# HydraRadio/hydra-pspec

Measured on NVIDIA B200. Metric: baseline-Gibbs-iterations/sec at Nfreq=384, Ntimes=1024, Nfg=32 on 1/8 B200, higher is better.
Workload: dtype f64 (complex128)

## Files before the change

### hydra_pspec_b200/_lib.py

```python
import ctypes as C
import os
from pathlib import Path

import numpy as np

_HERE = Path(__file__).resolve().parent
LIB_PATH = Path(os.environ.get("HP_LIB_PATH", _HERE / "csrc" / "libhydra_pspec_b200.so"))

HP_RNG_INJECTED, HP_RNG_PHILOX = 0, 1
HP_KEEP_CR, HP_KEEP_FG, HP_KEEP_CHISQ = 1, 2, 4
(HP_BUF_PS, HP_BUF_LNPOST, HP_BUF_CR, HP_BUF_FG, HP_BUF_CHISQ, HP_BUF_LAST_CR, HP_BUF_LAST_FG,
 HP_BUF_PS_CUR) = range(8)
HP_NUM_KERNEL_CLASSES = 6
HP_SUMMARY_CR, HP_SUMMARY_FG = 1, 2


class HPConfig(C.Structure):
    _fields_ = [
        ("device", C.c_int), ("nchains", C.c_int), ("ntimes", C.c_int), ("nfreqs", C.c_int),
        ("nmodes", C.c_int), ("rng_mode", C.c_int), ("cg_compat", C.c_int), ("refresh_omega", C.c_int),
        ("keep", C.c_int), ("max_iters", C.c_int), ("general_basis0", C.c_int), ("profile", C.c_int), ("substreams", C.c_int), ("dense_noise", C.c_int),
        ("force_dense_transforms", C.c_int), ("force_dense_solve", C.c_int), ("time_flags", C.c_int),
        ("ring_iters", C.c_int), ("seed", C.c_uint64), ("stream", C.c_void_p),
    ]
# ... 31 lines not shown
    "hp_engine_kernel_ms": (C.c_int, [C.c_void_p, C.c_void_p, C.c_void_p, C.c_int]),
    "hp_engine_set_substreams": (C.c_int, [C.c_void_p, C.c_int]),
    "hp_engine_set_chain_ids": (C.c_int, [C.c_void_p, C.c_void_p]),
    "hp_engine_set_profile": (C.c_int, [C.c_void_p, C.c_int]),
    "hp_engine_launch_count": (C.c_longlong, [C.c_void_p]),
    "hp_engine_set_summary": (C.c_int, [C.c_void_p, C.c_int, C.c_int, C.c_int]),
    "hp_engine_read_summary": (C.c_int, [C.c_void_p, C.c_int, C.c_int, C.c_void_p, C.c_void_p, C.c_size_t,
                                         C.POINTER(C.c_int)]),
    "hp_engine_set_summary_batched": (C.c_int, [C.c_void_p, C.c_int, C.c_int, C.c_int, C.c_int]),
    "hp_engine_read_summary_mcse": (C.c_int, [C.c_void_p, C.c_int, C.c_int, C.c_void_p, C.c_void_p, C.c_size_t,
                                              C.POINTER(C.c_int)]),
    "hp_engine_pt_form": (C.c_int, [C.c_void_p, C.POINTER(C.c_int), C.POINTER(C.c_int)]),
    "hp_kernel_class_name": (C.c_char_p, [C.c_int]),
    "hp_sample_S": (C.c_int, [C.c_int, C.c_int, C.c_int, C.c_void_p, C.c_void_p, C.c_void_p, C.c_void_p]),
    "hp_fourier_operator": (C.c_int, [C.c_int, C.c_int, C.c_void_p]),
    "hp_eigh_batch": (C.c_int, [C.c_int, C.c_int, C.c_int, C.c_void_p, C.c_void_p, C.c_void_p, C.c_void_p]),
    "hp_test_zgemm": (C.c_int, [C.c_int, C.c_int, C.c_int, C.c_void_p, C.c_int, C.c_int, C.c_void_p, C.c_int,
                                C.c_int, C.c_void_p, C.c_void_p]),
    "hp_test_chol_solve": (C.c_int, [C.c_int, C.c_int, C.c_int, C.c_void_p, C.c_void_p, C.c_void_p, C.c_void_p,
                                     C.c_int, C.c_void_p, C.c_void_p, C.c_void_p]),
    "hp_test_solve3": (C.c_int, [C.c_int, C.c_int, C.c_int, C.c_int, C.c_void_p, C.c_void_p, C.c_void_p, C.c_void_p,
                                 C.c_int, C.c_int, C.c_void_p, C.c_void_p]),
    "hp_test_solve3_schedule": (C.c_int, [C.c_int, C.c_void_p, C.c_void_p, C.POINTER(C.c_int), C.POINTER(C.c_int)]),
    "hp_fp64_peak_tflops": (C.c_double, [C.c_int, C.c_double]),
    "hp_release_cached_memory": (None, []),
    "hp_pinned_alloc": (C.c_void_p, [C.c_size_t]),
    "hp_pinned_free": (None, [C.c_void_p]),
    "hp_last_error": (C.c_char_p, []),
    "hp_version": (C.c_char_p, []),
}
EXPORTED_SYMBOLS = tuple(_SIGNATURES)


def lib():
    global _lib
    if _lib is None:
        if not LIB_PATH.exists():
            raise HydraLibError(
                f"{LIB_PATH} not found: build it with hydra_pspec_b200/csrc/build.sh "
                "(hydra_pspec_b200 has no CPU fallback)")
        L = C.CDLL(os.fspath(LIB_PATH))
        for name, (res, args) in _SIGNATURES.items():
            fn = getattr(L, name)
            fn.restype = res
            fn.argtypes = args
        _lib = L
# ... 66 lines not shown
```

### hydra_pspec_b200/csrc/hp_engine.cu

```cuda
#include "../../include/hydra_pspec_b200.h"
#include "hp_kernels.cuh"
#include "hp_math.h"

#include <cmath>
#include <cstdio>
#include <cstdlib>
#include <cstring>
#include <mutex>
#include <string>
#include <vector>

namespace {

thread_local std::string g_err;

int fail(int code, const std::string& msg) {
    g_err = msg;
    return code;
}

#define CU_TRY(expr)                                                                              \
    do {                                                                                          \
        cudaError_t _e = (expr);                                                                  \
        if (_e != cudaSuccess)                                                                    \
// ... 1040 lines not shown
        t.B = OFFS(b.Bmat, 2 * n * Np); t.sBk = 1; t.sBj = e->Np; t.bsB = (long long)e->n * e->Np;
        t.C = sf; t.sCi = e->n; t.sCj = 1; t.bsC = o.sf_bs;
        t.M = e->T; t.N = e->n; t.K = e->n; t.accumulate = 0; t.alpha = 1.0; t.batch = sb.nc;
        hp::launch_zgemm(t, sb.st);
        e->prof_end(CLS_TRANSFORM, 1, sb.st);
    }
    e->last_sf = o.sf;
    e->last_sf_bs = o.sf_bs;
    double* fg = o.fg ? o.fg + (size_t)sb.c0 * (size_t)o.fg_bs : nullptr;
    double* chisq = o.chisq ? o.chisq + (size_t)sb.c0 * (size_t)o.chisq_bs : nullptr;

    if (e->fft_ok) {
        e->prof_begin(CLS_POST, sb.st);
        hp::PostFftArgs pa{};
        pa.plan = e->plan; pa.tw = e->tw; pa.tw2 = e->tw2; pa.X = OFFS(e->X, 2 * Tp * Np); pa.lam = OFFS(e->lam, Np); pa.Sf = sf; pa.sf_bs = o.sf_bs;
        pa.Ft = OFFS(e->Ft, 2 * (m ? m : 1) * n); pa.wd = OFFS(e->wd, 2 * Tp * n); pa.w = OFFS(e->w, n); pa.ninvd = OFFS(e->ninvd, n);
        pa.w_bs = e->n; pa.w_ts = 0;
        if (pt) { pa.w = OFFS(e->wT, Tp * n); pa.w_bs = (long long)e->Tp * e->n; pa.w_ts = e->n; }
        pa.fg_out = fg; pa.fg_bs = o.fg_bs; pa.chisq_out = chisq; pa.chisq_bs = o.chisq_bs;
        pa.lnp1 = OFFS(e->lnp1, Tp); pa.Rm = e->cfg.dense_noise ? OFFS(e->Rm, 2 * Tp * n) : nullptr;
        pa.Empart = e->any_flagged ? OFFS(e->Empart, (size_t)e->ntilesE * n) : nullptr;
        pa.Eupart = general ? OFFS(e->Eupart, (size_t)e->ntilesE * n) : nullptr;
        pa.m = e->m; pa.Np = e->Np; pa.T = e->T; pa.Tp = e->Tp; pa.nsys = sb.nc; pa.do_inverse = fused_inverse ? 1 : 0; pa.ktp = e->ktp;
        if (!(e->fft2_ok && pa.do_inverse && !pa.Eupart && hp::launch_post_fft2(pa, e->plan2f, e->plan2r, sb.st)))
            hp::launch_post_fft(pa, sb.st);
        e->prof_end(CLS_POST, 1, sb.st);
        if (e->cfg.dense_noise) enqueue_dense_lnp1(e, sb);
        return;
    }
    e->prof_begin(CLS_POST, sb.st);
    hp::PostArgs pa{};
    pa.Sf = sf; pa.sf_bs = o.sf_bs; pa.X = OFFS(e->X, 2 * Tp * Np); pa.Ft = OFFS(e->Ft, 2 * (m ? m : 1) * n);
    pa.wd = OFFS(e->wd, 2 * Tp * n); pa.w = OFFS(e->w, n); pa.ninvd = OFFS(e->ninvd, n);
    pa.fg_out = fg; pa.fg_bs = o.fg_bs; pa.chisq_out = chisq; pa.chisq_bs = o.chisq_bs;
    pa.Wm = e->any_flagged ? OFFS(e->Wm, 2 * Tp * n) : nullptr; pa.Rm = e->cfg.dense_noise ? OFFS(e->Rm, 2 * Tp * n) : nullptr;
    pa.lnp1 = OFFS(e->lnp1, Tp);
    pa.n = e->n; pa.m = e->m; pa.Np = e->Np; pa.T = e->T; pa.Tp = e->Tp; pa.nsys = sb.nc;
    hp::launch_post(pa, sb.st);
    e->prof_end(CLS_POST, 1, sb.st);
    if (e->cfg.dense_noise) enqueue_dense_lnp1(e, sb);
    if (e->any_flagged || general) {
        e->prof_begin(CLS_TRANSFORM, sb.st);
        int nl2 = 0;
        hp::ZgemmArgs t{};
        t.sAi = e->n; t.sAk = 1; t.bsA = (long long)e->Tp * e->n;
        t.B = e->U; t.sBk = 1; t.sBj = e->n; t.bsB = 0;
// ... 575 lines not shown
```

### hydra_pspec_b200/csrc/hp_fft2.cu

```cuda
#include "hp_kernels.cuh"
#include "hp_math.h"
#include "hp_mma.cuh"
#include <cstdlib>

namespace hp {

namespace {

constexpr int kTP2 = 8;
#ifndef HP_FFT2_CTAS
#define HP_FFT2_CTAS 2
#endif

__device__ __forceinline__ double2 cmul(double2 a, double2 b) { return make_double2(a.x * b.x - a.y * b.y, a.x * b.y + a.y * b.x); }
__device__ __forceinline__ double2 cadd(double2 a, double2 b) { return make_double2(a.x + b.x, a.y + b.y); }
__device__ __forceinline__ double2 csub(double2 a, double2 b) { return make_double2(a.x - b.x, a.y - b.y); }
__device__ __forceinline__ double2 mul_mi(double2 a) { return make_double2(a.y, -a.x); }

template <int R>
__device__ __forceinline__ void butterfly(double2* a);
template <>
__device__ __forceinline__ void butterfly<2>(double2* a) {
    const double2 t = a[1];
    a[1] = csub(a[0], t);
    a[0] = cadd(a[0], t);
}
template <>
__device__ __forceinline__ void butterfly<3>(double2* a) {
    const double S3 = 0.86602540378443864676;
    const double2 t1 = cadd(a[1], a[2]);
    const double2 t2 = make_double2(a[0].x - 0.5 * t1.x, a[0].y - 0.5 * t1.y);
    const double2 t3 = make_double2(S3 * (a[1].y - a[2].y), -S3 * (a[1].x - a[2].x));
// ... 9 lines not shown
template <>
__device__ __forceinline__ void butterfly<6>(double2* a) {
    double2 e[3] = {a[0], a[2], a[4]}, o[3] = {a[3], a[5], a[1]};
    butterfly<3>(e);
    butterfly<3>(o);
    a[0] = cadd(e[0], o[0]); a[3] = csub(e[0], o[0]);
    a[4] = cadd(e[1], o[1]); a[1] = csub(e[1], o[1]);
    a[2] = cadd(e[2], o[2]); a[5] = csub(e[2], o[2]);
}
template <>
__device__ __forceinline__ void butterfly<8>(double2* a) {
    const double H = 0.70710678118654752440;
    double2 e[4] = {a[0], a[2], a[4], a[6]}, o[4] = {a[1], a[3], a[5], a[7]};
    butterfly<4>(e);
    butterfly<4>(o);
    const double2 o1 = make_double2(H * (o[1].x + o[1].y), H * (o[1].y - o[1].x));
    const double2 o2 = mul_mi(o[2]);
    const double2 o3 = make_double2(H * (o[3].y - o[3].x), -H * (o[3].x + o[3].y));
    a[0] = cadd(e[0], o[0]); a[4] = csub(e[0], o[0]);
    a[1] = cadd(e[1], o1);   a[5] = csub(e[1], o1);
    a[2] = cadd(e[2], o2);   a[6] = csub(e[2], o2);
    a[3] = cadd(e[3], o3);   a[7] = csub(e[3], o3);
}

__device__ __forceinline__ int phys(int i) { return i + (i >> 3); }

template <int E, int R, int NS, bool kLoad, bool kStore>
__device__ __forceinline__ void fft_pass(double2 (&v)[E], double2* row, const double2* __restrict__ twt, int lane) {
    constexpr int n = 32 * E, NB = E / R, nb = n / R;
    static_assert(E % R == 0 && nb % 8 == 0, "a lane owns whole butterflies; rows of a butterfly are 8-aligned");
    if (kLoad) {
        const double2* src = row + phys(lane);
#pragma unroll
        for (int u = 0; u < NB; ++u)
#pragma unroll
            for (int r = 0; r < R; ++r) v[u * R + r] = src[36 * u + r * (nb / 8 * 9)];
    }
#pragma unroll
    for (int u = 0; u < NB; ++u) {
        if (NS > 1) {
            const int k = (lane + 32 * u) % NS;
#pragma unroll
            for (int r = 1; r < R; ++r) v[u * R + r] = cmul(v[u * R + r], twt[k * (R - 1) + r - 1]);
        }
        butterfly<R>(&v[u * R]);
    }
// ... 50 lines not shown
    else if (n == 512) { rad[0] = 8; rad[1] = 8; rad[2] = 4; rad[3] = 2; nf = 4; }
    else if (n == 256) { rad[0] = 8; rad[1] = 8; rad[2] = 4; rad[3] = 1; nf = 3; }
    else if (n == 128) { rad[0] = 4; rad[1] = 4; rad[2] = 4; rad[3] = 2; nf = 4; }
    else return false;
    for (int dir = 0; dir < 2; ++dir) {
        FftPlan* p = dir ? rev : fwd;
        p->n = n; p->nf = nf;
        int Ns = 1;
        for (int i = 0; i < nf; ++i) {
            p->radix[i] = dir ? rad[nf - 1 - i] : rad[i];
            p->magic[i] = Ns > 1 ? (uint32_t)((0x100000000ull + (uint64_t)Ns - 1) / (uint64_t)Ns) : 0u;
            Ns *= p->radix[i];
        }
    }
    return true;
}

size_t postfft2_smem_bytes(int n, int m) {
    const int mk = ((m + 3) / 4) * 4;
    const int ld = n + n / 8 + 1;
    return sizeof(double2) * ((size_t)kTP2 * ld + 2 * (size_t)n + (size_t)kTP2 * (((mk + 7) / 8) * 8 + 4)) + 80 * sizeof(double);
}

template <int E, int P0, int P1, int P2, int P3>
__global__ void __launch_bounds__(32 * kTP2, (E >= 16 ? 1 : HP_FFT2_CTAS)) k_post_fft2(PostFftArgs a) {
    constexpr int kThreads = 32 * kTP2;
    constexpr int n = 32 * E, ld = n + n / 8 + 1;
    constexpr int RL = P3 > 1 ? P3 : P2;
    extern __shared__ __align__(16) unsigned char smem_raw[];
    const int m = a.m, mk = ((m + 3) / 4) * 4, ldf = ((mk + 7) / 8) * 8 + 4;
    double2* A = reinterpret_cast<double2*>(smem_raw);
    double2* tw = A + (size_t)kTP2 * ld;
    double2* fs = tw + 2 * (size_t)n;
    double* red = reinterpret_cast<double*>(fs + (size_t)kTP2 * ldf);
    const int sys = blockIdx.y, tile = blockIdx.x, t0 = tile * kTP2;
    const int tid = threadIdx.x, warp = tid >> 5, lane = tid & 31;
    const double* X = a.X + 2 * ((size_t)sys * a.Tp + t0) * a.Np;
    const double* lam = a.lam + (size_t)sys * a.Np;
    const double* w = a.w + (size_t)sys * a.w_bs + (size_t)t0 * a.w_ts;
    const double* nd = a.ninvd + (size_t)sys * n;
    const double* wd = a.wd + 2 * ((size_t)sys * a.Tp + t0) * n;
    double* Sf = a.Sf + 2 * ((size_t)sys * a.sf_bs + (size_t)t0 * n);
    const double2* twg = reinterpret_cast<const double2*>(a.tw);
    const double rsn = rsqrt((double)n);

    {
        const char* wdp = reinterpret_cast<const char*>(wd);
        const size_t bytes = (size_t)min(kTP2, a.T - t0) * n * 16;
        for (size_t off = (size_t)tid * 128; off < bytes; off += kThreads * 128) asm volatile("prefetch.global.L2 [%0];" ::"l"(wdp + off));
    }
    const int t = warp;
    const bool live = t0 + t < a.T;
    double2 v[E];
    {
        constexpr int nb0 = n / P0;
        const double* xr = X + 2 * (size_t)t * a.Np;
#pragma unroll
        for (int e = 0; e < E; ++e) {
            const int u = e / P0, r = e - u * P0;
            const int k = lane + 32 * u + r * nb0;
            double2 y = make_double2(0.0, 0.0);
            double l = 0.0;
            if (live) { y = *reinterpret_cast<const double2*>(xr + 2 * k); l = lam[k]; }
            const double sg = (k & 1) ? -l : l;
            v[e] = make_double2(sg * y.x, -sg * y.y);
        }
    }
    if (a.tw2) {
        const double2* t2 = reinterpret_cast<const double2*>(a.tw2);
        const int cnt = a.Empart ? 2 * n : n;
        for (int e = tid; e < cnt; e += kThreads) tw[e] = t2[e];
    } else {
        build_twiddle_tables<E, P0, P1, P2, P3>(tw, twg, tid, kThreads);
        if (a.Empart) {
            if constexpr (P3 > 1) build_twiddle_tables<E, P3, P2, P1, P0>(tw + n, twg, tid, kThreads);
            else build_twiddle_tables<E, P2, P1, P0, 1>(tw + n, twg, tid, kThreads);
        }
    }
    for (int e = tid; e < kTP2 * ldf; e += kThreads) {
        const int tt = e / ldf, j = e - tt * ldf;
        double2 f = make_double2(0.0, 0.0);
        if (j < m && t0 + tt < a.T) f = *reinterpret_cast<const double2*>(X + 2 * ((size_t)tt * a.Np + n + j));
        fs[e] = f;
        if (j < m && t0 + tt < a.T && a.fg_out)
            *reinterpret_cast<double2*>(a.fg_out + (size_t)sys * a.fg_bs + 2 * ((size_t)(t0 + tt) * m + j)) = f;
    }
    __syncthreads();
    double2* row = A + (size_t)t * ld;
    {
        fft_run<E, P0, P1, P2, P3, true>(v, row, tw, lane);
        constexpr int R = RL, Ns = n / RL;
        const double2 c0 = twg[(int)(((long long)(n / 2) * (n / 2)) % n)];
        __syncwarp();
#pragma unroll
        for (int e = 0; e < E; ++e) {
            const int u = e / R, r = e - u * R;
            const int x = lane + 32 * u + r * Ns;
            double2 o = cmul(v[e], c0);
            const double sg = (x & 1) ? -rsn : rsn;
            o = make_double2(sg * o.x, -sg * o.y);
            row[phys(x)] = o;
            if (live) *reinterpret_cast<double2*>(Sf + 2 * ((size_t)t * n + x)) = o;
        }
    }
    __syncthreads();
    {
        const double* Ft = a.Ft + 2 * (size_t)sys * m * n;
        const int nct = n / 8;
        const int g = lane >> 2, q = lane & 3;
        const bool tlive = t0 + g < a.T;
        const double* wrow = w + (size_t)g * a.w_ts;
        double lnp = 0.0;
        constexpr int kBF = 8;
        double2 bnx[kBF], dnx[2];
        auto load_tile = [&](int ct, double2 (&b)[kBF], double2 (&d)[2]) {
            const int x = 8 * ct + g;
#pragma unroll
            for (int s8 = 0; s8 < kBF; ++s8) {
                const int k = 4 * s8 + q;
                b[s8] = (k < m && ct < nct) ? *reinterpret_cast<const double2*>(Ft + 2 * ((size_t)k * n + x)) : make_double2(0.0, 0.0);
            }
            d[0] = d[1] = make_double2(0.0, 0.0);
            if (tlive && ct < nct) {
                d[0] = *reinterpret_cast<const double2*>(wd + 2 * ((size_t)g * n + 8 * ct + 2 * q));
                d[1] = *reinterpret_cast<const double2*>(wd + 2 * ((size_t)g * n + 8 * ct + 2 * q + 1));
            }
        };
        load_tile(warp, bnx, dnx);
        for (int ct = warp; ct < nct; ct += kTP2) {
            double p1[2] = {0.0, 0.0}, p2[2] = {0.0, 0.0}, p3[2] = {0.0, 0.0};
            const int x0 = 8 * ct + 2 * q;
            double2 bc[kBF];
#pragma unroll
            for (int s8 = 0; s8 < kBF; ++s8) bc[s8] = bnx[s8];
            const double2 d0 = dnx[0], d1 = dnx[1];
            load_tile(ct + kTP2, bnx, dnx);
#pragma unroll
            for (int s8 = 0; s8 < kBF; ++s8) {
                const int k = 4 * s8 + q;
                if (4 * s8 < mk) {
                    const double2 af = fs[(size_t)g * ldf + k];
                    dmma884(p1[0], p1[1], af.x, bc[s8].x);
                    dmma884(p2[0], p2[1], af.y, bc[s8].y);
                    dmma884(p3[0], p3[1], af.x + af.y, bc[s8].x + bc[s8].y);
                }
            }
            for (int kc = 4 * kBF; kc < mk; kc += 4) {
                const int k = kc + q;
                const double2 af = fs[(size_t)g * ldf + k];
                const double2 b = k < m ? *reinterpret_cast<const double2*>(Ft + 2 * ((size_t)k * n + 8 * ct + g)) : make_double2(0.0, 0.0);
                dmma884(p1[0], p1[1], af.x, b.x);
                dmma884(p2[0], p2[1], af.y, b.y);
                dmma884(p3[0], p3[1], af.x + af.y, b.x + b.y);
            }
            const double2 s0 = A[(size_t)g * ld + phys(x0)], s1 = A[(size_t)g * ld + phys(x0 + 1)];
            const double wx0 = (a.w_ts == 0 || tlive) ? wrow[x0] : 0.0, wx1 = (a.w_ts == 0 || tlive) ? wrow[x0 + 1] : 0.0;
            const double n0 = nd[x0], n1 = nd[x0 + 1];
            const double rr0 = d0.x - s0.x - (p1[0] - p2[0]), ri0 = d0.y - s0.y - (p3[0] - p1[0] - p2[0]);
            const double rr1 = d1.x - s1.x - (p1[1] - p2[1]), ri1 = d1.y - s1.y - (p3[1] - p1[1] - p2[1]);
            const double q0 = rr0 * rr0 + ri0 * ri0, q1 = rr1 * rr1 + ri1 * ri1;
            if (tlive) {
                if (a.chisq_out)
                    *reinterpret_cast<double2*>(a.chisq_out + (size_t)sys * a.chisq_bs + (size_t)(t0 + g) * n + x0) = make_double2(q0 * n0, q1 * n1);
                lnp += wx0 * n0 * q0 + wx1 * n1 * q1;
                if (a.Rm) {
                    double* rm = a.Rm + 2 * (((size_t)sys * a.Tp + t0 + g) * n + x0);
                    *reinterpret_cast<double2*>(rm) = make_double2(wx0 * rr0, wx0 * ri0);
                    *reinterpret_cast<double2*>(rm + 2) = make_double2(wx1 * rr1, wx1 * ri1);
                }
            }
            if (a.Empart) {
                A[(size_t)g * ld + phys(x0)] = make_double2(wx0 * s0.x, wx0 * s0.y);
                A[(size_t)g * ld + phys(x0 + 1)] = make_double2(-wx1 * s1.x, -wx1 * s1.y);
            }
        }
        lnp += __shfl_xor_sync(0xffffffffu, lnp, 1);
        lnp += __shfl_xor_sync(0xffffffffu, lnp, 2);
        if (q == 0) red[warp * kTP2 + g] = lnp;
    }
    __syncthreads();
    if (tid < kTP2) {
        double s = 0.0;
        for (int wv = 0; wv < kTP2; ++wv) s += red[wv * kTP2 + tid];
        if (t0 + tid < a.Tp) a.lnp1[(size_t)sys * a.Tp + t0 + tid] = t0 + tid < a.T ? s : 0.0;
    }
    if (a.Empart) {
        if constexpr (P3 > 1) fft_run<E, P3, P2, P1, P0, false>(v, row, tw + n, lane);
        else fft_run<E, P2, P1, P0, 1, false>(v, row, tw + n, lane);
        constexpr int R = P0, Ns = n / P0;
        __syncwarp();
        double* erow = reinterpret_cast<double*>(row);
#pragma unroll
        for (int e = 0; e < E; ++e) {
            const int u = e / R, r = e - u * R;
            erow[lane + 32 * u + r * Ns] = live ? v[e].x * v[e].x + v[e].y * v[e].y : 0.0;
        }
        __syncthreads();
        double* Ep = a.Empart + ((size_t)sys * gridDim.x + tile) * n;
        for (int k = tid; k < n; k += kThreads) {
            double acc = 0.0;
#pragma unroll
            for (int tt = 0; tt < kTP2; ++tt) acc += reinterpret_cast<const double*>(A + (size_t)tt * ld)[k];
            Ep[k] = acc / (double)n;
        }
    }
}

namespace {
template <int E, int P0, int P1, int P2, int P3>
__global__ void __launch_bounds__(256) k_fft2_tables(double2* tw2, const double2* twg) {
    constexpr int n = 32 * E;
    for (int e = threadIdx.x; e < 2 * n; e += 256) tw2[e] = make_double2(0.0, 0.0);
    __syncthreads();
    build_twiddle_tables<E, P0, P1, P2, P3>(tw2, twg, threadIdx.x, 256);
    if constexpr (P3 > 1) build_twiddle_tables<E, P3, P2, P1, P0>(tw2 + n, twg, threadIdx.x, 256);
    else build_twiddle_tables<E, P2, P1, P0, 1>(tw2 + n, twg, threadIdx.x, 256);
}
}

bool launch_fft2_tables(double* tw2, const double* tw, int n, cudaStream_t st) {
    double2* o = reinterpret_cast<double2*>(tw2);
    const double2* t = reinterpret_cast<const double2*>(tw);
    if (n == 128) k_fft2_tables<4, 4, 4, 4, 2><<<1, 256, 0, st>>>(o, t);
    else if (n == 256) k_fft2_tables<8, 8, 8, 4, 1><<<1, 256, 0, st>>>(o, t);
    else if (n == 384) k_fft2_tables<12, 6, 4, 4, 4><<<1, 256, 0, st>>>(o, t);
    else if (n == 512) k_fft2_tables<16, 8, 8, 4, 2><<<1, 256, 0, st>>>(o, t);
    else if (n == 1024) k_fft2_tables<32, 8, 8, 4, 4><<<1, 256, 0, st>>>(o, t);
    else return false;
    return true;
}

bool launch_post_fft2(const PostFftArgs& a, const FftPlan& fwd, const FftPlan& rev, cudaStream_t st) {
    (void)rev;
    const int n = fwd.n;
    const size_t smem = postfft2_smem_bytes(n, a.m);
    static size_t attr_dev[kMaxDev][5] = {{0}};
    const int slot = n == 128 ? 0 : (n == 256 ? 1 : (n == 384 ? 2 : (n == 512 ? 3 : 4)));
    size_t& attr = attr_dev[current_device_slot()][slot];
    const dim3 grid((a.T + kTP2 - 1) / kTP2, a.nsys);
    if (n == 128) {
        if (smem > attr) { cudaFuncSetAttribute(k_post_fft2<4, 4, 4, 4, 2>, cudaFuncAttributeMaxDynamicSharedMemorySize, (int)smem); attr = smem; }
        k_post_fft2<4, 4, 4, 4, 2><<<grid, 32 * kTP2, smem, st>>>(a);
    } else if (n == 256) {
        if (smem > attr) { cudaFuncSetAttribute(k_post_fft2<8, 8, 8, 4, 1>, cudaFuncAttributeMaxDynamicSharedMemorySize, (int)smem); attr = smem; }
        k_post_fft2<8, 8, 8, 4, 1><<<grid, 32 * kTP2, smem, st>>>(a);
    } else if (n == 384) {
        if (smem > attr) { cudaFuncSetAttribute(k_post_fft2<12, 6, 4, 4, 4>, cudaFuncAttributeMaxDynamicSharedMemorySize, (int)smem); attr = smem; }
        k_post_fft2<12, 6, 4, 4, 4><<<grid, 32 * kTP2, smem, st>>>(a);
    } else if (n == 512) {
        if (smem > attr) { cudaFuncSetAttribute(k_post_fft2<16, 8, 8, 4, 2>, cudaFuncAttributeMaxDynamicSharedMemorySize, (int)smem); attr = smem; }
        k_post_fft2<16, 8, 8, 4, 2><<<grid, 32 * kTP2, smem, st>>>(a);
    } else if (n == 1024) {
        if (smem > attr) { cudaFuncSetAttribute(k_post_fft2<32, 8, 8, 4, 4>, cudaFuncAttributeMaxDynamicSharedMemorySize, (int)smem); attr = smem; }
        k_post_fft2<32, 8, 8, 4, 4><<<grid, 32 * kTP2, smem, st>>>(a);
    } else {
        return false;
    }
    return true;
}

}
```

### hydra_pspec_b200/csrc/hp_kernels.cuh

```cuda
#pragma once
#include <cuda_runtime.h>
#include <stdint.h>

namespace hp {

constexpr int kNB = 32;
constexpr int kBlkDoubles = 2 * 32 * 32;
constexpr int kLdBlk = 36;
constexpr int kLPlane = 32 * kLdBlk;
constexpr int kLBlkDoubles = 2 * kLPlane;
constexpr int kTT = 16;
constexpr int kInvGrid = 1000;

constexpr int kMaxDev = 64;
inline int current_device_slot() {
    int d = 0;
    cudaGetDevice(&d);
    return (d < 0 || d >= kMaxDev) ? 0 : d;
}

__host__ __device__ inline size_t tri_blocks(int nblk) { return (size_t)nblk * (nblk + 1) / 2; }
__host__ __device__ inline size_t blk_index(int i, int j) { return (size_t)i * (i + 1) / 2 + j; }

struct ZgemmArgs {
// ... 166 lines not shown
void launch_twiddles(double* tw, int n, cudaStream_t st);
int postfft_ktp(int n, int m, size_t max_smem);
int postfft_tiles(int T, int ktp);
size_t postfft_smem_bytes(int n, int m, int ktp);

struct PostFftArgs {
    FftPlan plan;
    const double* tw;
    const double* tw2;
    const double* X;
    const double* lam;
    double* Sf;
    long long sf_bs;
    const double* Ft;
    const double* wd; const double* w; const double* ninvd;
    long long w_bs, w_ts;
    double* fg_out; double* chisq_out; long long fg_bs, chisq_bs;
    double* lnp1;
    double* Rm;
    double* Empart;
    double* Eupart;
    int m, Np, T, Tp, nsys, do_inverse;
    int ktp;
};
void launch_post_fft(const PostFftArgs& a, cudaStream_t st);
bool make_fft2_plan(int n, FftPlan* fwd, FftPlan* rev);
size_t postfft2_smem_bytes(int n, int m);
bool launch_post_fft2(const PostFftArgs& a, const FftPlan& fwd, const FftPlan& rev, cudaStream_t st);
bool launch_fft2_tables(double* tw2, const double* tw, int n, cudaStream_t st);

struct MomentsArr {
    const double* src; long long src_cs; int w, rs;
    int L, nsys; long long ld;
    double* mean; double* m2;
};
int launch_moments(const MomentsArr& cr, const MomentsArr& fg, double invk, cudaStream_t st);
struct MomentsBatch {
    double* snap; double* m2;
};
int launch_moments_batch(const MomentsArr& cr, const MomentsArr& fg, const MomentsBatch& crb, const MomentsBatch& fgb,
                         double invk, double jj1, cudaStream_t st);

}
```

### hydra_pspec_b200/csrc/hp_testhooks.cu

```cuda
#include "../../include/hydra_pspec_b200.h"
#include "hp_kernels.cuh"

#include <string>
#include <vector>

extern "C" {

int hp_test_zgemm(int M, int N, int K, const double* A, int transA, int conjA, const double* B, int transB, int conjB,
                  const double* dk, double* C) {
    double *dA, *dB, *dC, *dD = nullptr;
    if (cudaMalloc(&dA, 16ull * M * K) || cudaMalloc(&dB, 16ull * K * N) || cudaMalloc(&dC, 16ull * M * N)) return HP_ERR_CUDA;
    cudaMemcpy(dA, A, 16ull * M * K, cudaMemcpyHostToDevice);
    cudaMemcpy(dB, B, 16ull * K * N, cudaMemcpyHostToDevice);
    if (dk) { cudaMalloc(&dD, 8ull * K); cudaMemcpy(dD, dk, 8ull * K, cudaMemcpyHostToDevice); }
    hp::ZgemmArgs g{};
    g.A = dA; g.sAi = transA ? 1 : K; g.sAk = transA ? M : 1; g.conjA = conjA;
    g.B = dB; g.sBk = transB ? 1 : N; g.sBj = transB ? K : 1; g.conjB = conjB;
    g.C = dC; g.sCi = N; g.sCj = 1; g.dk = dD;
    g.M = M; g.N = N; g.K = K; g.alpha = 1.0; g.batch = 1;
    hp::launch_zgemm(g, 0);
    cudaError_t e = cudaDeviceSynchronize();
    cudaMemcpy(C, dC, 16ull * M * N, cudaMemcpyDeviceToHost);
    cudaFree(dA); cudaFree(dB); cudaFree(dC); cudaFree(dD);
    return e == cudaSuccess ? HP_OK : HP_ERR_CUDA;
// ... 113 lines not shown
                    psum[(size_t)s * n + k] = acc;
                }
        }
    }
    cudaFree(dG); cudaFree(dGp); cudaFree(dlam); cudaFree(dLp); cudaFree(dLinv); cudaFree(dWp); cudaFree(dR);
    cudaFree(dW); cudaFree(dX); cudaFree(dP); cudaFree(dinfo); cudaFree(dRt); cudaFree(dWf1); cudaFree(dWf2);
    return e == cudaSuccess ? HP_OK : HP_ERR_CUDA;
}

int hp_test_solve3_schedule(int nblk, unsigned char* n, unsigned char* strips, int* nwarps, int* max_per_warp) {
    if (nblk < 1 || 2 * nblk > hp::kS3MaxStrips) return HP_ERR_SIZE;
    hp::Solve3Sched sc{};
    hp::solve3_make_schedule(nblk, &sc);
    for (int p = 0; p < 2; ++p)
        for (int w = 0; w < hp::kS3Warps; ++w) {
            n[p * hp::kS3Warps + w] = sc.n[p][w];
            for (int e = 0; e < hp::kS3MaxPerWarp; ++e) strips[(p * hp::kS3Warps + w) * hp::kS3MaxPerWarp + e] = sc.strip[p][w][e];
        }
    *nwarps = hp::kS3Warps;
    *max_per_warp = hp::kS3MaxPerWarp;
    return HP_OK;
}

namespace {
__global__ void __launch_bounds__(256) k_fp64_peak(double* out, int iters, double a, double b) {
    double c[8][2];
#pragma unroll
    for (int i = 0; i < 8; ++i) { c[i][0] = threadIdx.x; c[i][1] = i; }
    for (int it = 0; it < iters; ++it) {
#pragma unroll
        for (int i = 0; i < 8; ++i)
            asm volatile("mma.sync.aligned.m8n8k4.row.col.f64.f64.f64.f64 {%0,%1}, {%2}, {%3}, {%0,%1};"
                         : "+d"(c[i][0]), "+d"(c[i][1]) : "d"(a), "d"(b));
    }
    double s = 0;
#pragma unroll
    for (int i = 0; i < 8; ++i) s += c[i][0] + c[i][1];
    if (s == 12345.678) out[0] = s;
}
}

double hp_fp64_peak_tflops(int device, double seconds) {
    if (cudaSetDevice(device) != cudaSuccess) return -1.0;
    int nsm = 0;
    cudaDeviceGetAttribute(&nsm, cudaDevAttrMultiProcessorCount, device);
    double* out;
// ... 31 lines not shown
```

### include/hydra_pspec_b200.h

```cpp
#ifndef HYDRA_PSPEC_B200_H
#define HYDRA_PSPEC_B200_H

#include <stddef.h>
#include <stdint.h>

#ifdef __cplusplus
extern "C" {
#endif

typedef struct hp_engine hp_engine;

enum hp_status { HP_OK = 0, HP_ERR_ARG = -1, HP_ERR_CUDA = -2, HP_ERR_SIZE = -3, HP_ERR_NUMERIC = -4 };

enum hp_rng_mode {
    HP_RNG_INJECTED = 0,
    HP_RNG_PHILOX = 1
};

enum hp_keep { HP_KEEP_CR = 1, HP_KEEP_FG = 2, HP_KEEP_CHISQ = 4 };

enum hp_buffer {
    HP_BUF_PS = 0,
    HP_BUF_LNPOST = 1,
    HP_BUF_CR = 2,
// ... 68 lines not shown
int hp_engine_info(hp_engine* e, int* info_host);

int hp_engine_kernel_ms(hp_engine* e, double* ms, int* launches, int reset);
int hp_engine_set_chain_ids(hp_engine* e, const int* ids);
int hp_engine_set_substreams(hp_engine* e, int n);
int hp_engine_set_profile(hp_engine* e, int on);
int hp_engine_pt_form(const hp_engine* e, int* low_rank, int* max_rank);
long long hp_engine_launch_count(const hp_engine* e);

int hp_sample_S(int device, int ntimes, int nfreqs, const double* s, const double* prior, const double* draws,
                double* out);

int hp_fourier_operator(int device, int n, double* out);
int hp_eigh_batch(int device, int n, int batch, const double* S, double* V, double* w, int* sweeps);

int hp_test_zgemm(int M, int N, int K, const double* A, int transA, int conjA, const double* B, int transB, int conjB,
                  const double* dk, double* C);
int hp_test_chol_solve(int n, int m, int T, const double* G, const double* lam, const double* Rfix, const double* wa,
                       int cg_compat, double* Ldense, double* X, int* info);
int hp_test_solve3(int n, int m, int T, int nsys, const double* G, const double* lam, const double* Rfix, const double* wa,
                   int cg_compat, int grid_limit, double* X, double* psum);

int hp_test_solve3_schedule(int nblk, unsigned char* n, unsigned char* strips, int* nwarps, int* max_per_warp);

double hp_fp64_peak_tflops(int device, double seconds);
void hp_release_cached_memory(void);
void* hp_pinned_alloc(size_t bytes);
void hp_pinned_free(void* p);

const char* hp_last_error(void);
const char* hp_version(void);

#ifdef __cplusplus
}
#endif
#endif
```

Measured before the change: 16580.

## Make post-FFT2 kernel persistent grid-stride over tiles with next-item L2 prefetch

Converts the k_post_fft2 kernel from one CTA per (tile, system) to a persistent grid sized from occupancy that walks work items in a grid-stride loop (for E<32), prefetching the next item's X and wd rows into L2 while it processes the current one. Twiddle tables are built once per CTA instead of once per tile. The intent is to amortise per-CTA setup and hide global load latency. In exchange, each CTA now does serial work and there is extra loop overhead. The change also adds optional clock64 timers and a test hook that caps the grid size.

```diff
diff --git a/hydra_pspec_b200/_lib.py b/hydra_pspec_b200/_lib.py
--- a/hydra_pspec_b200/_lib.py
+++ b/hydra_pspec_b200/_lib.py
@@ -77,6 +77,7 @@
     "hp_test_solve3": (C.c_int, [C.c_int, C.c_int, C.c_int, C.c_int, C.c_void_p, C.c_void_p, C.c_void_p, C.c_void_p,
                                  C.c_int, C.c_int, C.c_void_p, C.c_void_p]),
     "hp_test_solve3_schedule": (C.c_int, [C.c_int, C.c_void_p, C.c_void_p, C.POINTER(C.c_int), C.POINTER(C.c_int)]),
+    "hp_test_set_post2_grid_limit": (None, [C.c_int]),
     "hp_fp64_peak_tflops": (C.c_double, [C.c_int, C.c_double]),
     "hp_release_cached_memory": (None, []),
     "hp_pinned_alloc": (C.c_void_p, [C.c_size_t]),
diff --git a/hydra_pspec_b200/csrc/hp_engine.cu b/hydra_pspec_b200/csrc/hp_engine.cu
--- a/hydra_pspec_b200/csrc/hp_engine.cu
+++ b/hydra_pspec_b200/csrc/hp_engine.cu
@@ -1086,6 +1086,7 @@
         pa.Empart = e->any_flagged ? OFFS(e->Empart, (size_t)e->ntilesE * n) : nullptr;
         pa.Eupart = general ? OFFS(e->Eupart, (size_t)e->ntilesE * n) : nullptr;
         pa.m = e->m; pa.Np = e->Np; pa.T = e->T; pa.Tp = e->Tp; pa.nsys = sb.nc; pa.do_inverse = fused_inverse ? 1 : 0; pa.ktp = e->ktp;
+        pa.grid_limit = hp::g_post2_grid_limit;
         if (!(e->fft2_ok && pa.do_inverse && !pa.Eupart && hp::launch_post_fft2(pa, e->plan2f, e->plan2r, sb.st)))
             hp::launch_post_fft(pa, sb.st);
         e->prof_end(CLS_POST, 1, sb.st);
diff --git a/hydra_pspec_b200/csrc/hp_fft2.cu b/hydra_pspec_b200/csrc/hp_fft2.cu
--- a/hydra_pspec_b200/csrc/hp_fft2.cu
+++ b/hydra_pspec_b200/csrc/hp_fft2.cu
@@ -8,6 +8,7 @@
 namespace {
 
 constexpr int kTP2 = 8;
+template <int E> constexpr bool kWalk = E < 32;
 #ifndef HP_FFT2_CTAS
 #define HP_FFT2_CTAS 2
 #endif
@@ -63,6 +64,8 @@
     a[2] = cadd(e[2], o2);   a[6] = csub(e[2], o2);
     a[3] = cadd(e[3], o3);   a[7] = csub(e[3], o3);
 }
+
+__device__ __forceinline__ int thread_x() { int v; asm volatile("mov.u32 %0, %%tid.x;" : "=r"(v)); return v; }
 
 __device__ __forceinline__ int phys(int i) { return i + (i >> 3); }
 
@@ -159,8 +162,25 @@
     return sizeof(double2) * ((size_t)kTP2 * ld + 2 * (size_t)n + (size_t)kTP2 * (((mk + 7) / 8) * 8 + 4)) + 80 * sizeof(double);
 }
 
+__device__ unsigned long long g_post2_cycles[10];
+#ifdef HP_POST2_TIMERS
+#define P2_T(idx) do { const long long now_ = clock64(); tacc[idx] += now_ - tlast; tlast = now_; } while (0)
+#else
+#define P2_T(idx) do { } while (0)
+#endif
+
+extern "C" void hp_post2_timers(unsigned long long* out, int reset) {
+    cudaDeviceSynchronize();
+    cudaMemcpyFromSymbol(out, g_post2_cycles, sizeof(unsigned long long) * 10);
+    if (reset) { unsigned long long z[10] = {0}; cudaMemcpyToSymbol(g_post2_cycles, z, sizeof(z)); }
+}
+
 template <int E, int P0, int P1, int P2, int P3>
 __global__ void __launch_bounds__(32 * kTP2, (E >= 16 ? 1 : HP_FFT2_CTAS)) k_post_fft2(PostFftArgs a) {
+#ifdef HP_POST2_TIMERS
+    long long tacc[10] = {0, 0, 0, 0, 0, 0, 0, 0, 0, 0}, tlast = clock64();
+    const long long tstart = tlast;
+#endif
     constexpr int kThreads = 32 * kTP2;
     constexpr int n = 32 * E, ld = n + n / 8 + 1;
     constexpr int RL = P3 > 1 ? P3 : P2;
@@ -170,39 +190,20 @@
     double2* tw = A + (size_t)kTP2 * ld;
     double2* fs = tw + 2 * (size_t)n;
     double* red = reinterpret_cast<double*>(fs + (size_t)kTP2 * ldf);
-    const int sys = blockIdx.y, tile = blockIdx.x, t0 = tile * kTP2;
-    const int tid = threadIdx.x, warp = tid >> 5, lane = tid & 31;
-    const double* X = a.X + 2 * ((size_t)sys * a.Tp + t0) * a.Np;
-    const double* lam = a.lam + (size_t)sys * a.Np;
-    const double* w = a.w + (size_t)sys * a.w_bs + (size_t)t0 * a.w_ts;
-    const double* nd = a.ninvd + (size_t)sys * n;
-    const double* wd = a.wd + 2 * ((size_t)sys * a.Tp + t0) * n;
-    double* Sf = a.Sf + 2 * ((size_t)sys * a.sf_bs + (size_t)t0 * n);
+    const int tid = threadIdx.x;
+    const int ntiles = (a.T + kTP2 - 1) / kTP2, items = ntiles * a.nsys;
     const double2* twg = reinterpret_cast<const double2*>(a.tw);
-    const double rsn = rsqrt((double)n);
-
-    {
-        const char* wdp = reinterpret_cast<const char*>(wd);
-        const size_t bytes = (size_t)min(kTP2, a.T - t0) * n * 16;
-        for (size_t off = (size_t)tid * 128; off < bytes; off += kThreads * 128) asm volatile("prefetch.global.L2 [%0];" ::"l"(wdp + off));
-    }
-    const int t = warp;
-    const bool live = t0 + t < a.T;
-    double2 v[E];
-    {
-        constexpr int nb0 = n / P0;
-        const double* xr = X + 2 * (size_t)t * a.Np;
-#pragma unroll
-        for (int e = 0; e < E; ++e) {
-            const int u = e / P0, r = e - u * P0;
-            const int k = lane + 32 * u + r * nb0;
-            double2 y = make_double2(0.0, 0.0);
-            double l = 0.0;
-            if (live) { y = *reinterpret_cast<const double2*>(xr + 2 * k); l = lam[k]; }
-            const double sg = (k & 1) ? -l : l;
-            v[e] = make_double2(sg * y.x, -sg * y.y);
-        }
-    }
+
+    auto prefetch_item = [&](int it) {
+        if (it >= items) return;
+        const int s = it / ntiles, tn = (it - s * ntiles) * kTP2, rows = min(kTP2, a.T - tn);
+        const char* xp = reinterpret_cast<const char*>(a.X + 2 * ((size_t)s * a.Tp + tn) * a.Np);
+        const char* dp = reinterpret_cast<const char*>(a.wd + 2 * ((size_t)s * a.Tp + tn) * n);
+        const size_t xb = (size_t)rows * a.Np * 16, db = (size_t)rows * n * 16;
+        for (size_t off = (size_t)tid * 128; off < xb; off += kThreads * 128) asm volatile("prefetch.global.L2 [%0];" ::"l"(xp + off));
+        for (size_t off = (size_t)tid * 128; off < db; off += kThreads * 128) asm volatile("prefetch.global.L2 [%0];" ::"l"(dp + off));
+    };
+    prefetch_item(blockIdx.x);
     if (a.tw2) {
         const double2* t2 = reinterpret_cast<const double2*>(a.tw2);
         const int cnt = a.Empart ? 2 * n : n;
@@ -214,133 +215,178 @@
             else build_twiddle_tables<E, P2, P1, P0, 1>(tw + n, twg, tid, kThreads);
         }
     }
-    for (int e = tid; e < kTP2 * ldf; e += kThreads) {
-        const int tt = e / ldf, j = e - tt * ldf;
-        double2 f = make_double2(0.0, 0.0);
-        if (j < m && t0 + tt < a.T) f = *reinterpret_cast<const double2*>(X + 2 * ((size_t)tt * a.Np + n + j));
-        fs[e] = f;
-        if (j < m && t0 + tt < a.T && a.fg_out)
-            *reinterpret_cast<double2*>(a.fg_out + (size_t)sys * a.fg_bs + 2 * ((size_t)(t0 + tt) * m + j)) = f;
-    }
-    __syncthreads();
-    double2* row = A + (size_t)t * ld;
-    {
-        fft_run<E, P0, P1, P2, P3, true>(v, row, tw, lane);
-        constexpr int R = RL, Ns = n / RL;
-        const double2 c0 = twg[(int)(((long long)(n / 2) * (n / 2)) % n)];
-        __syncwarp();
-#pragma unroll
-        for (int e = 0; e < E; ++e) {
-            const int u = e / R, r = e - u * R;
-            const int x = lane + 32 * u + r * Ns;
-            double2 o = cmul(v[e], c0);
-            const double sg = (x & 1) ? -rsn : rsn;
-            o = make_double2(sg * o.x, -sg * o.y);
-            row[phys(x)] = o;
-            if (live) *reinterpret_cast<double2*>(Sf + 2 * ((size_t)t * n + x)) = o;
-        }
-    }
-    __syncthreads();
-    {
-        const double* Ft = a.Ft + 2 * (size_t)sys * m * n;
-        const int nct = n / 8;
-        const int g = lane >> 2, q = lane & 3;
-        const bool tlive = t0 + g < a.T;
-        const double* wrow = w + (size_t)g * a.w_ts;
-        double lnp = 0.0;
-        constexpr int kBF = 8;
-        double2 bnx[kBF], dnx[2];
-        auto load_tile = [&](int ct, double2 (&b)[kBF], double2 (&d)[2]) {
-            const int x = 8 * ct + g;
-#pragma unroll
-            for (int s8 = 0; s8 < kBF; ++s8) {
-                const int k = 4 * s8 + q;
-                b[s8] = (k < m && ct < nct) ? *reinterpret_cast<const double2*>(Ft + 2 * ((size_t)k * n + x)) : make_double2(0.0, 0.0);
+
+    for (int it = blockIdx.x; it < items; it = kWalk<E> ? it + (int)gridDim.x : items) {
+        const int tid = thread_x(), warp = tid >> 5, lane = tid & 31;
+        const int sys = it / ntiles, tile = it - sys * ntiles, t0 = tile * kTP2;
+        const double* X = a.X + 2 * ((size_t)sys * a.Tp + t0) * a.Np;
+        const double* lam = a.lam + (size_t)sys * a.Np;
+        const double* w = a.w + (size_t)sys * a.w_bs + (size_t)t0 * a.w_ts;
+        const double* nd = a.ninvd + (size_t)sys * n;
+        const double* wd = a.wd + 2 * ((size_t)sys * a.Tp + t0) * n;
+        double* Sf = a.Sf + 2 * ((size_t)sys * a.sf_bs + (size_t)t0 * n);
+        prefetch_item(it + gridDim.x);
+        const int t = warp;
+        const bool live = t0 + t < a.T;
+        double2 v[E];
+        {
+            constexpr int nb0 = n / P0;
+            const double* xr = X + 2 * (size_t)t * a.Np;
+#pragma unroll
+            for (int e = 0; e < E; ++e) {
+                const int u = e / P0, r = e - u * P0;
+                const int k = lane + 32 * u + r * nb0;
+                double2 y = make_double2(0.0, 0.0);
+                double l = 0.0;
+                if (live) { y = *reinterpret_cast<const double2*>(xr + 2 * k); l = lam[k]; }
+                const double sg = (k & 1) ? -l : l;
+                v[e] = make_double2(sg * y.x, -sg * y.y);
             }
-            d[0] = d[1] = make_double2(0.0, 0.0);
-            if (tlive && ct < nct) {
-                d[0] = *reinterpret_cast<const double2*>(wd + 2 * ((size_t)g * n + 8 * ct + 2 * q));
-                d[1] = *reinterpret_cast<const double2*>(wd + 2 * ((size_t)g * n + 8 * ct + 2 * q + 1));
+        }
+        for (int e = tid; e < kTP2 * ldf; e += kThreads) {
+            const int tt = e / ldf, j = e - tt * ldf;
+            double2 f = make_double2(0.0, 0.0);
+            if (j < m && t0 + tt < a.T) f = *reinterpret_cast<const double2*>(X + 2 * ((size_t)tt * a.Np + n + j));
+            fs[e] = f;
+            if (j < m && t0 + tt < a.T && a.fg_out)
+                *reinterpret_cast<double2*>(a.fg_out + (size_t)sys * a.fg_bs + 2 * ((size_t)(t0 + tt) * m + j)) = f;
+        }
+        P2_T(0);
+        __syncthreads();
+        P2_T(1);
+        double2* row = A + (size_t)t * ld;
+        {
+            fft_run<E, P0, P1, P2, P3, true>(v, row, tw, lane);
+            constexpr int R = RL, Ns = n / RL;
+            const double rsn = rsqrt((double)n);
+            const double2 c0 = twg[(int)(((long long)(n / 2) * (n / 2)) % n)];
+            __syncwarp();
+#pragma unroll
+            for (int e = 0; e < E; ++e) {
+                const int u = e / R, r = e - u * R;
+                const int x = lane + 32 * u + r * Ns;
+                double2 o = cmul(v[e], c0);
+                const double sg = (x & 1) ? -rsn : rsn;
+                o = make_double2(sg * o.x, -sg * o.y);
+                row[phys(x)] = o;
+                if (live) *reinterpret_cast<double2*>(Sf + 2 * ((size_t)t * n + x)) = o;
             }
-        };
-        load_tile(warp, bnx, dnx);
-        for (int ct = warp; ct < nct; ct += kTP2) {
-            double p1[2] = {0.0, 0.0}, p2[2] = {0.0, 0.0}, p3[2] = {0.0, 0.0};
-            const int x0 = 8 * ct + 2 * q;
-            double2 bc[kBF];
-#pragma unroll
-            for (int s8 = 0; s8 < kBF; ++s8) bc[s8] = bnx[s8];
-            const double2 d0 = dnx[0], d1 = dnx[1];
-            load_tile(ct + kTP2, bnx, dnx);
-#pragma unroll
-            for (int s8 = 0; s8 < kBF; ++s8) {
-                const int k = 4 * s8 + q;
-                if (4 * s8 < mk) {
+        }
+        P2_T(2);
+        __syncthreads();
+        P2_T(3);
+        {
+            const double* Ft = a.Ft + 2 * (size_t)sys * m * n;
+            const int nct = n / 8;
+            const int g = lane >> 2, q = lane & 3;
+            const bool tlive = t0 + g < a.T;
+            const double* wrow = w + (size_t)g * a.w_ts;
+            double lnp = 0.0;
+            constexpr int kBF = 8;
+            double2 bnx[kBF], dnx[2];
+            auto load_tile = [&](int ct, double2 (&b)[kBF], double2 (&d)[2]) {
+                const int x = 8 * ct + g;
+#pragma unroll
+                for (int s8 = 0; s8 < kBF; ++s8) {
+                    const int k = 4 * s8 + q;
+                    b[s8] = (k < m && ct < nct) ? *reinterpret_cast<const double2*>(Ft + 2 * ((size_t)k * n + x)) : make_double2(0.0, 0.0);
+                }
+                d[0] = d[1] = make_double2(0.0, 0.0);
+                if (tlive && ct < nct) {
+                    d[0] = *reinterpret_cast<const double2*>(wd + 2 * ((size_t)g * n + 8 * ct + 2 * q));
+                    d[1] = *reinterpret_cast<const double2*>(wd + 2 * ((size_t)g * n + 8 * ct + 2 * q + 1));
+                }
+            };
+            load_tile(warp, bnx, dnx);
+            for (int ct = warp; ct < nct; ct += kTP2) {
+                double p1[2] = {0.0, 0.0}, p2[2] = {0.0, 0.0}, p3[2] = {0.0, 0.0};
+                const int x0 = 8 * ct + 2 * q;
+                double2 bc[kBF];
+#pragma unroll
+                for (int s8 = 0; s8 < kBF; ++s8) bc[s8] = bnx[s8];
+                const double2 d0 = dnx[0], d1 = dnx[1];
+                load_tile(ct + kTP2, bnx, dnx);
+#pragma unroll
+                for (int s8 = 0; s8 < kBF; ++s8) {
+                    const int k = 4 * s8 + q;
+                    if (4 * s8 < mk) {
+                        const double2 af = fs[(size_t)g * ldf + k];
+                        dmma884(p1[0], p1[1], af.x, bc[s8].x);
+                        dmma884(p2[0], p2[1], af.y, bc[s8].y);
+                        dmma884(p3[0], p3[1], af.x + af.y, bc[s8].x + bc[s8].y);
+                    }
+                }
+                for (int kc = 4 * kBF; kc < mk; kc += 4) {
+                    const int k = kc + q;
                     const double2 af = fs[(size_t)g * ldf + k];
-                    dmma884(p1[0], p1[1], af.x, bc[s8].x);
-                    dmma884(p2[0], p2[1], af.y, bc[s8].y);
-                    dmma884(p3[0], p3[1], af.x + af.y, bc[s8].x + bc[s8].y);
+                    const double2 b = k < m ? *reinterpret_cast<const double2*>(Ft + 2 * ((size_t)k * n + 8 * ct + g)) : make_double2(0.0, 0.0);
+                    dmma884(p1[0], p1[1], af.x, b.x);
+                    dmma884(p2[0], p2[1], af.y, b.y);
+                    dmma884(p3[0], p3[1], af.x + af.y, b.x + b.y);
+                }
+                const double2 s0 = A[(size_t)g * ld + phys(x0)], s1 = A[(size_t)g * ld + phys(x0 + 1)];
+                const double wx0 = (a.w_ts == 0 || tlive) ? wrow[x0] : 0.0, wx1 = (a.w_ts == 0 || tlive) ? wrow[x0 + 1] : 0.0;
+                const double n0 = nd[x0], n1 = nd[x0 + 1];
+                const double rr0 = d0.x - s0.x - (p1[0] - p2[0]), ri0 = d0.y - s0.y - (p3[0] - p1[0] - p2[0]);
+                const double rr1 = d1.x - s1.x - (p1[1] - p2[1]), ri1 = d1.y - s1.y - (p3[1] - p1[1] - p2[1]);
+                const double q0 = rr0 * rr0 + ri0 * ri0, q1 = rr1 * rr1 + ri1 * ri1;
+                if (tlive) {
+                    if (a.chisq_out)
+                        *reinterpret_cast<double2*>(a.chisq_out + (size_t)sys * a.chisq_bs + (size_t)(t0 + g) * n + x0) = make_double2(q0 * n0, q1 * n1);
+                    lnp += wx0 * n0 * q0 + wx1 * n1 * q1;
+                    if (a.Rm) {
+                        double* rm = a.Rm + 2 * (((size_t)sys * a.Tp + t0 + g) * n + x0);
+                        *reinterpret_cast<double2*>(rm) = make_double2(wx0 * rr0, wx0 * ri0);
+                        *reinterpret_cast<double2*>(rm + 2) = make_double2(wx1 * rr1, wx1 * ri1);
+                    }
+                }
+                if (a.Empart) {
+                    A[(size_t)g * ld + phys(x0)] = make_double2(wx0 * s0.x, wx0 * s0.y);
+                    A[(size_t)g * ld + phys(x0 + 1)] = make_double2(-wx1 * s1.x, -wx1 * s1.y);
                 }
             }
-            for (int kc = 4 * kBF; kc < mk; kc += 4) {
-                const int k = kc + q;
-                const double2 af = fs[(size_t)g * ldf + k];
-                const double2 b = k < m ? *reinterpret_cast<const double2*>(Ft + 2 * ((size_t)k * n + 8 * ct + g)) : make_double2(0.0, 0.0);
-                dmma884(p1[0], p1[1], af.x, b.x);
-                dmma884(p2[0], p2[1], af.y, b.y);
-                dmma884(p3[0], p3[1], af.x + af.y, b.x + b.y);
+            lnp += __shfl_xor_sync(0xffffffffu, lnp, 1);
+            lnp += __shfl_xor_sync(0xffffffffu, lnp, 2);
+            if (q == 0) red[warp * kTP2 + g] = lnp;
+        }
+        P2_T(4);
+        __syncthreads();
+        P2_T(5);
+        if (tid < kTP2) {
+            double s = 0.0;
+            for (int wv = 0; wv < kTP2; ++wv) s += red[wv * kTP2 + tid];
+            if (t0 + tid < a.Tp) a.lnp1[(size_t)sys * a.Tp + t0 + tid] = t0 + tid < a.T ? s : 0.0;
+        }
+        P2_T(6);
+        if (a.Empart) {
+            if constexpr (P3 > 1) fft_run<E, P3, P2, P1, P0, false>(v, row, tw + n, lane);
+            else fft_run<E, P2, P1, P0, 1, false>(v, row, tw + n, lane);
+            constexpr int R = P0, Ns = n / P0;
+            __syncwarp();
+            double* erow = reinterpret_cast<double*>(row);
+#pragma unroll
+            for (int e = 0; e < E; ++e) {
+                const int u = e / R, r = e - u * R;
+                erow[lane + 32 * u + r * Ns] = live ? v[e].x * v[e].x + v[e].y * v[e].y : 0.0;
             }
-            const double2 s0 = A[(size_t)g * ld + phys(x0)], s1 = A[(size_t)g * ld + phys(x0 + 1)];
-            const double wx0 = (a.w_ts == 0 || tlive) ? wrow[x0] : 0.0, wx1 = (a.w_ts == 0 || tlive) ? wrow[x0 + 1] : 0.0;
-            const double n0 = nd[x0], n1 = nd[x0 + 1];
-            const double rr0 = d0.x - s0.x - (p1[0] - p2[0]), ri0 = d0.y - s0.y - (p3[0] - p1[0] - p2[0]);
-            const double rr1 = d1.x - s1.x - (p1[1] - p2[1]), ri1 = d1.y - s1.y - (p3[1] - p1[1] - p2[1]);
-            const double q0 = rr0 * rr0 + ri0 * ri0, q1 = rr1 * rr1 + ri1 * ri1;
-            if (tlive) {
-                if (a.chisq_out)
-                    *reinterpret_cast<double2*>(a.chisq_out + (size_t)sys * a.chisq_bs + (size_t)(t0 + g) * n + x0) = make_double2(q0 * n0, q1 * n1);
-                lnp += wx0 * n0 * q0 + wx1 * n1 * q1;
-                if (a.Rm) {
-                    double* rm = a.Rm + 2 * (((size_t)sys * a.Tp + t0 + g) * n + x0);
-                    *reinterpret_cast<double2*>(rm) = make_double2(wx0 * rr0, wx0 * ri0);
-                    *reinterpret_cast<double2*>(rm + 2) = make_double2(wx1 * rr1, wx1 * ri1);
-                }
+            P2_T(6);
+            __syncthreads();
+            P2_T(7);
+            double* Ep = a.Empart + ((size_t)sys * ntiles + tile) * n;
+            for (int k = tid; k < n; k += kThreads) {
+                double acc = 0.0;
+#pragma unroll
+                for (int tt = 0; tt < kTP2; ++tt) acc += reinterpret_cast<const double*>(A + (size_t)tt * ld)[k];
+                Ep[k] = acc / (double)n;
             }
-            if (a.Empart) {
-                A[(size_t)g * ld + phys(x0)] = make_double2(wx0 * s0.x, wx0 * s0.y);
-                A[(size_t)g * ld + phys(x0 + 1)] = make_double2(-wx1 * s1.x, -wx1 * s1.y);
-            }
-        }
-        lnp += __shfl_xor_sync(0xffffffffu, lnp, 1);
-        lnp += __shfl_xor_sync(0xffffffffu, lnp, 2);
-        if (q == 0) red[warp * kTP2 + g] = lnp;
-    }
-    __syncthreads();
-    if (tid < kTP2) {
-        double s = 0.0;
-        for (int wv = 0; wv < kTP2; ++wv) s += red[wv * kTP2 + tid];
-        if (t0 + tid < a.Tp) a.lnp1[(size_t)sys * a.Tp + t0 + tid] = t0 + tid < a.T ? s : 0.0;
-    }
-    if (a.Empart) {
-        if constexpr (P3 > 1) fft_run<E, P3, P2, P1, P0, false>(v, row, tw + n, lane);
-        else fft_run<E, P2, P1, P0, 1, false>(v, row, tw + n, lane);
-        constexpr int R = P0, Ns = n / P0;
-        __syncwarp();
-        double* erow = reinterpret_cast<double*>(row);
-#pragma unroll
-        for (int e = 0; e < E; ++e) {
-            const int u = e / R, r = e - u * R;
-            erow[lane + 32 * u + r * Ns] = live ? v[e].x * v[e].x + v[e].y * v[e].y : 0.0;
-        }
-        __syncthreads();
-        double* Ep = a.Empart + ((size_t)sys * gridDim.x + tile) * n;
-        for (int k = tid; k < n; k += kThreads) {
-            double acc = 0.0;
-#pragma unroll
-            for (int tt = 0; tt < kTP2; ++tt) acc += reinterpret_cast<const double*>(A + (size_t)tt * ld)[k];
-            Ep[k] = acc / (double)n;
-        }
-    }
+            P2_T(8);
+        }
+    }
+#ifdef HP_POST2_TIMERS
+    tacc[9] = clock64() - tstart;
+    if ((tid & 31) == 0)
+        for (int i = 0; i < 10; ++i) atomicAdd(&g_post2_cycles[i], (unsigned long long)tacc[i]);
+#endif
 }
 
 namespace {
@@ -367,32 +413,41 @@
     return true;
 }
 
+int g_post2_grid_limit = 0;
+
+namespace {
+template <int E, int P0, int P1, int P2, int P3>
+void launch_walk(const PostFftArgs& a, size_t smem, int slot, cudaStream_t st) {
+    auto kern = k_post_fft2<E, P0, P1, P2, P3>;
+    struct Resident { size_t smem, attr; int grid; };
+    static Resident res_dev[kMaxDev][5] = {};
+    Resident& r = res_dev[current_device_slot()][slot];
+    if (smem > r.attr) { cudaFuncSetAttribute(kern, cudaFuncAttributeMaxDynamicSharedMemorySize, (int)smem); r.attr = smem; }
+    if (smem != r.smem) {
+        int dev = 0, nsm = 0, per_sm = 0;
+        cudaGetDevice(&dev);
+        cudaDeviceGetAttribute(&nsm, cudaDevAttrMultiProcessorCount, dev);
+        cudaOccupancyMaxActiveBlocksPerMultiprocessor(&per_sm, kern, 32 * kTP2, smem);
+        r.grid = (per_sm > 0 ? per_sm : 1) * nsm;
+        r.smem = smem;
+    }
+    const int items = (a.T + kTP2 - 1) / kTP2 * a.nsys;
+    int grid = !kWalk<E> ? items : (a.grid_limit > 0 ? a.grid_limit : r.grid);
+    if (grid > items) grid = items;
+    kern<<<grid, 32 * kTP2, smem, st>>>(a);
+}
+}
+
 bool launch_post_fft2(const PostFftArgs& a, const FftPlan& fwd, const FftPlan& rev, cudaStream_t st) {
     (void)rev;
     const int n = fwd.n;
     const size_t smem = postfft2_smem_bytes(n, a.m);
-    static size_t attr_dev[kMaxDev][5] = {{0}};
-    const int slot = n == 128 ? 0 : (n == 256 ? 1 : (n == 384 ? 2 : (n == 512 ? 3 : 4)));
-    size_t& attr = attr_dev[current_device_slot()][slot];
-    const dim3 grid((a.T + kTP2 - 1) / kTP2, a.nsys);
-    if (n == 128) {
-        if (smem > attr) { cudaFuncSetAttribute(k_post_fft2<4, 4, 4, 4, 2>, cudaFuncAttributeMaxDynamicSharedMemorySize, (int)smem); attr = smem; }
-        k_post_fft2<4, 4, 4, 4, 2><<<grid, 32 * kTP2, smem, st>>>(a);
-    } else if (n == 256) {
-        if (smem > attr) { cudaFuncSetAttribute(k_post_fft2<8, 8, 8, 4, 1>, cudaFuncAttributeMaxDynamicSharedMemorySize, (int)smem); attr = smem; }
-        k_post_fft2<8, 8, 8, 4, 1><<<grid, 32 * kTP2, smem, st>>>(a);
-    } else if (n == 384) {
-        if (smem > attr) { cudaFuncSetAttribute(k_post_fft2<12, 6, 4, 4, 4>, cudaFuncAttributeMaxDynamicSharedMemorySize, (int)smem); attr = smem; }
-        k_post_fft2<12, 6, 4, 4, 4><<<grid, 32 * kTP2, smem, st>>>(a);
-    } else if (n == 512) {
-        if (smem > attr) { cudaFuncSetAttribute(k_post_fft2<16, 8, 8, 4, 2>, cudaFuncAttributeMaxDynamicSharedMemorySize, (int)smem); attr = smem; }
-        k_post_fft2<16, 8, 8, 4, 2><<<grid, 32 * kTP2, smem, st>>>(a);
-    } else if (n == 1024) {
-        if (smem > attr) { cudaFuncSetAttribute(k_post_fft2<32, 8, 8, 4, 4>, cudaFuncAttributeMaxDynamicSharedMemorySize, (int)smem); attr = smem; }
-        k_post_fft2<32, 8, 8, 4, 4><<<grid, 32 * kTP2, smem, st>>>(a);
-    } else {
-        return false;
-    }
+    if (n == 128) launch_walk<4, 4, 4, 4, 2>(a, smem, 0, st);
+    else if (n == 256) launch_walk<8, 8, 8, 4, 1>(a, smem, 1, st);
+    else if (n == 384) launch_walk<12, 6, 4, 4, 4>(a, smem, 2, st);
+    else if (n == 512) launch_walk<16, 8, 8, 4, 2>(a, smem, 3, st);
+    else if (n == 1024) launch_walk<32, 8, 8, 4, 4>(a, smem, 4, st);
+    else return false;
     return true;
 }
 
diff --git a/hydra_pspec_b200/csrc/hp_kernels.cuh b/hydra_pspec_b200/csrc/hp_kernels.cuh
--- a/hydra_pspec_b200/csrc/hp_kernels.cuh
+++ b/hydra_pspec_b200/csrc/hp_kernels.cuh
@@ -212,11 +212,13 @@
     double* Eupart;
     int m, Np, T, Tp, nsys, do_inverse;
     int ktp;
+    int grid_limit;
 };
 void launch_post_fft(const PostFftArgs& a, cudaStream_t st);
 bool make_fft2_plan(int n, FftPlan* fwd, FftPlan* rev);
 size_t postfft2_smem_bytes(int n, int m);
 bool launch_post_fft2(const PostFftArgs& a, const FftPlan& fwd, const FftPlan& rev, cudaStream_t st);
+extern int g_post2_grid_limit;
 bool launch_fft2_tables(double* tw2, const double* tw, int n, cudaStream_t st);
 
 struct MomentsArr {
diff --git a/hydra_pspec_b200/csrc/hp_testhooks.cu b/hydra_pspec_b200/csrc/hp_testhooks.cu
--- a/hydra_pspec_b200/csrc/hp_testhooks.cu
+++ b/hydra_pspec_b200/csrc/hp_testhooks.cu
@@ -159,6 +159,8 @@
     return HP_OK;
 }
 
+void hp_test_set_post2_grid_limit(int grid_limit) { hp::g_post2_grid_limit = grid_limit > 0 ? grid_limit : 0; }
+
 namespace {
 __global__ void __launch_bounds__(256) k_fp64_peak(double* out, int iters, double a, double b) {
     double c[8][2];
diff --git a/include/hydra_pspec_b200.h b/include/hydra_pspec_b200.h
--- a/include/hydra_pspec_b200.h
+++ b/include/hydra_pspec_b200.h
@@ -114,6 +114,7 @@
                    int cg_compat, int grid_limit, double* X, double* psum);
 
 int hp_test_solve3_schedule(int nblk, unsigned char* n, unsigned char* strips, int* nwarps, int* max_per_warp);
+void hp_test_set_post2_grid_limit(int grid_limit);
 
 double hp_fp64_peak_tflops(int device, double seconds);
 void hp_release_cached_memory(void);
```

New measurement: 16650, median of 6. No clear change (+0.4%).
